# danavery/audio-tokens

Measured on AMD Instinct MI355X. Metric: STFT frames/sec through K-means+tokenize, n_mels=64 vocab=8192, higher is better.
Workload: dtype f32; 1 GPU; configs[3] per-GPU shard x1: 22500+2500 clips/GPU of 10 s @22.05 kHz (43075000 frames/GPU), n_mels=64, vocab_size=8192, niter=20, k-means batches of 10000 files on a 2097152-row subsample; parallelism=dp1

## Files before the change

audio_tokens_amd/_lib.py:

```python
from __future__ import annotations

import ctypes
from pathlib import Path

_PKG = Path(__file__).resolve().parent
LIB_PATH = _PKG / "libaudio_tokens_amd.so"

AT_LAYOUT_MEL_MAJOR = 0
AT_LAYOUT_FRAME_MAJOR = 1

_c = ctypes
_vp, _i32, _i64 = _c.c_void_p, _c.c_int, _c.c_int64

class PrunedArgs(_c.Structure):
    _fields_ = [("x", _vp), ("n", _i64), ("d", _i32), ("c", _vp), ("k", _i32), ("order", _vp), ("hint_sorted", _vp),
                ("cperm", _vp), ("ng", _i32), ("bounds", _vp), ("guess_only", _i32), ("use_filter", _i32),
                ("prepass_done", _i32), ("image_current", _i32), ("ids", _vp), ("dist_or_null", _vp)]


SIGNATURES = {
    "at_version": (_i32, []),
    "at_last_error": (_c.c_char_p, []),
    "at_create": (_i32, [_i32, _c.POINTER(_vp)]),
    "at_destroy": (None, [_vp]),
    "at_workspace_bytes": (_i64, [_vp]),
    "at_background_stream": (_i32, [_vp, _c.POINTER(_vp)]),
    "at_debug_set": (_i32, [_vp, _c.c_char_p, _i32]),
    "at_debug_get": (_i32, [_vp, _c.c_char_p, _c.POINTER(_i32)]),
    "at_diag_errors": (_i32, [_c.POINTER(_i64), _c.POINTER(_i32), _c.POINTER(_i64), _c.POINTER(_i32), _c.c_char_p, _i32, _i32]),
    "at_debug_leave_error_pending": (_i32, []),
    "at_rand_perm_mt19937": (_i32, [_i64, _i64, _vp]),
    "at_rand_perm_prefix_mt19937": (_i32, [_i64, _i64, _i64, _vp]),
    "at_rand_perm_prefix_device": (_i32, [_vp, _i64, _i64, _i64, _vp, _vp]),
    "at_mel_filterbank_host": (_i32, [_i32, _i32, _i32, _vp]),
    "at_num_frames": (_i64, [_i64, _i32]),
    "at_split_clusters_host": (_i32, [_i32, _i32, _i64, _vp, _vp, _c.POINTER(_i32)]),
    "at_logmel_f32": (_i32, [_vp, _vp, _i64, _i64, _i64, _i32, _i32, _i32, _i32, _vp, _vp, _i32, _i32, _vp]),
    "at_resample_length": (_i64, [_i64, _i32, _i32]),
    "at_resample_taps_host": (_i32, [_i32, _i32, _c.POINTER(_i32), _c.POINTER(_i32), _c.POINTER(_i32), _vp, _i64]),
    "at_resample_f32": (_i32, [_vp, _vp, _i64, _i64, _i64, _i32, _i32, _vp, _i64, _vp]),
    "at_minmax_scale_clips_f32": (_i32, [_vp, _vp, _i64, _i64, _vp]),
    "at_conv1d_mel_f32": (_i32, [_vp, _vp, _i64, _i32, _vp, _vp, _i32, _i32, _i32, _vp, _vp]),
    "at_logmel_minmax_f32": (_i32, [_vp, _vp, _i64, _i64, _i64, _i32, _i32, _i32, _i32, _vp, _vp, _i32, _vp]),
    "at_l2norm_rows_f32": (_i32, [_vp, _vp, _i64, _i32, _vp, _vp]),
    "at_assign_f32": (_i32, [_vp, _vp, _i64, _i32, _vp, _i32, _vp, _vp, _vp]),
    "at_assign_hinted_f32": (_i32, [_vp, _vp, _i64, _i32, _vp, _i32, _vp, _vp, _vp, _vp, _vp, _vp]),
    "at_group_rows_kd_host": (_i32, [_vp, _i32, _i32, _i32, _vp]),
    "at_group_min_dist_f32": (_i32, [_vp, _vp, _i32, _i32, _vp, _i32, _vp, _vp]),
    "at_visit_order_f32": (_i32, [_vp, _vp, _vp, _i64, _i32, _vp, _vp, _vp]),
    "at_prune_stats": (_i32, [_vp, _c.POINTER(_i64), _c.POINTER(_i64), _i32]),
    "at_assign_coarse_f32": (_i32, [_vp, _vp, _i64, _i32, _vp, _i32, _vp, _i32, _vp, _vp, _vp, _vp, _vp]),
    "at_filter_stats": (_i32, [_vp, _c.POINTER(_i64), _c.POINTER(_i64), _c.POINTER(_c.c_double), _c.POINTER(_i64),
                               _c.POINTER(_i64), _c.POINTER(_i64), _i32]),
    "at_filter_probe_f32": (_i32, [_vp, _vp, _i64, _i32, _vp, _i32, _vp, _vp, _vp, _i32, _vp, _vp, _vp,
                                   _c.POINTER(_i64), _vp]),
    "at_group_means_f32": (_i32, [_vp, _vp, _i32, _i32, _vp, _i32, _vp, _vp]),
    "at_group_neighbours_f32": (_i32, [_vp, _vp, _i32, _i32, _i32, _vp, _vp]),
    "at_assign_pruned_f32": (_i32, [_vp, _vp, _vp]),
    "at_prune_mask_f32": (_i32, [_vp, _vp, _i64, _i32, _vp, _i32, _vp, _vp, _i32, _vp, _i32, _vp]),
    "at_gather_rows_f32": (_i32, [_vp, _vp, _i32, _vp, _i64, _vp, _vp]),
# ... 90 lines not shown
```

audio_tokens_amd/backend.py:

```python
from __future__ import annotations

import ctypes
import os

import numpy as np
import torch

from . import _lib

_vp = ctypes.c_void_p


def _ptr(t) -> _vp:
    return _vp(t.data_ptr()) if t is not None else _vp(None)


def _np_ptr(a: np.ndarray) -> _vp:
    return _vp(a.ctypes.data)


class HostHelpers:

    def __init__(self):
        self.lib = _lib.load()
# ... 160 lines not shown
        return torch.empty(shape, dtype=dtype).pin_memory()

    def synchronize(self) -> None:
        torch.cuda.current_stream(self.device).synchronize()

    def background_stream(self):
        if getattr(self, "_bg_stream", None) is None:
            h = ctypes.c_void_p()
            _lib.check(self.lib.at_background_stream(self.ctx.handle, ctypes.byref(h)))
            self._bg_stream = torch.cuda.ExternalStream(h.value, device=self.device)
        return self._bg_stream

    def record_event_timed(self):
        ev = torch.cuda.Event(enable_timing=True)
        ev.record(torch.cuda.current_stream(self.device))
        return ev

    def record_event(self):
        ev = torch.cuda.Event()
        ev.record(torch.cuda.current_stream(self.device))
        return ev

    def logmel(self, wave, sample_rate=22050, n_fft=512, hop=128, n_mels=64, fb=None,
               frame_major=False, l2norm=False, out=None) -> torch.Tensor:
        wave = self._f32(wave)
        if wave.dim() == 1:
            wave = wave.unsqueeze(0)
        assert wave.dim() == 2
        n_clips, L = wave.shape
        T = self.num_frames(L, hop)
        fbt = self._f32(fb) if fb is not None else None
        if fbt is not None:
            assert tuple(fbt.shape) == (n_fft // 2 + 1, n_mels), "fb must be [n_fft/2+1, n_mels]"
        shape = (n_clips * T, n_mels) if frame_major else (n_clips, n_mels, T)
        if out is None:
            out = self.empty(shape)
        else:
            assert out.is_contiguous() and out.dtype == torch.float32 and out.numel() == n_clips * T * n_mels
        rec = self._trace_list("logmel")
        if rec is not None:
            e0, e1 = torch.cuda.Event(enable_timing=True), torch.cuda.Event(enable_timing=True)
            e0.record(torch.cuda.current_stream(self.device))
        with torch.cuda.device(self.device):
            _lib.check(self.lib.at_logmel_f32(
                self.ctx.handle, _ptr(wave), n_clips, L, wave.stride(0), sample_rate, n_fft, hop, n_mels,
                _ptr(fbt), _ptr(out), _lib.AT_LAYOUT_FRAME_MAJOR if frame_major else _lib.AT_LAYOUT_MEL_MAJOR,
                1 if l2norm else 0, self._stream()))
        if rec is not None:
            e1.record(torch.cuda.current_stream(self.device))
            rec.append(("logmel", n_clips * T, n_mels, hop, e0, e1))
        return out

    def logmel_minmax(self, wave, sample_rate=22050, n_fft=512, hop=128, n_mels=64, fb=None) -> torch.Tensor:
        wave = self._f32(wave)
        if wave.dim() == 1:
            wave = wave.unsqueeze(0)
        n_clips, L = wave.shape
        T = self.num_frames(L, hop)
        fbt = self._f32(fb) if fb is not None else None
        out = self.empty((n_clips, n_mels, T))
        with torch.cuda.device(self.device):
            for c0 in range(0, n_clips, 65535):
                c1 = min(n_clips, c0 + 65535)
                _lib.check(self.lib.at_logmel_minmax_f32(
                    self.ctx.handle, _ptr(wave[c0:c1]), c1 - c0, L, wave.stride(0), sample_rate, n_fft, hop, n_mels,
                    _ptr(fbt), _ptr(out[c0:c1]), _lib.AT_LAYOUT_MEL_MAJOR, self._stream()))
        return out

    def resample(self, wave, orig_freq: int, new_freq: int) -> torch.Tensor:
        wave = self._f32(wave)
        squeeze = wave.dim() == 1
        if squeeze:
            wave = wave.unsqueeze(0)
# ... 446 lines not shown
```

audio_tokens_amd/csrc/host_group.cpp:

```cpp
#include <algorithm>
#include <cmath>
#include <vector>

#include "at_internal.h"

extern "C" {

int at_group_rows_kd_host(const float* rows, int k, int d, int leaf, int32_t* perm_out) {
    AT_REQUIRE(rows && perm_out && k > 0 && d > 0 && leaf > 0, "at_group_rows_kd_host: bad arguments");
    const int ngroups = (k + leaf - 1) / leaf;
    std::vector<int32_t> idx((size_t)k);
    for (int i = 0; i < k; i++) idx[i] = i;
    struct Part { int lo, hi, g0, g1; };
    std::vector<Part> stack{{0, k, 0, ngroups}};
    std::vector<int> bounds((size_t)ngroups + 1, 0);
    bounds[ngroups] = k;
    std::vector<float> meanf((size_t)d), axisf((size_t)d), nextf((size_t)d), proj((size_t)k), cen;
    while (!stack.empty()) {
        const Part p = stack.back();
        stack.pop_back();
        if (p.g1 - p.g0 <= 1) {
            bounds[p.g0] = p.lo;
            continue;
        }
// ... 9 lines not shown
            const float* r = rows + (size_t)idx[p.lo + i] * d;
            float* c = cen.data() + (size_t)i * d;
            for (int f = 0; f < d; f++) c[f] = r[f] - meanf[f];
        }
        for (int f = 0; f < d; f++) axisf[f] = 1.0f + 0.01f * (float)f;
        for (int it = 0; it < 4; it++) {
            std::fill(nextf.begin(), nextf.end(), 0.0f);
            for (int i = 0; i < m; i++) {
                const float* c = cen.data() + (size_t)i * d;
                float t = 0.0f;
                for (int f = 0; f < d; f++) t += c[f] * axisf[f];
                for (int f = 0; f < d; f++) nextf[f] += t * c[f];
            }
            float nrm = 0.0f;
            for (int f = 0; f < d; f++) nrm += nextf[f] * nextf[f];
            if (!(nrm > 0.0f)) break;
            nrm = 1.0f / std::sqrt(nrm);
            for (int f = 0; f < d; f++) axisf[f] = nextf[f] * nrm;
        }
        for (int i = 0; i < m; i++) {
            const float* c = cen.data() + (size_t)i * d;
            float t = 0.0f;
            for (int f = 0; f < d; f++) t += c[f] * axisf[f];
            proj[idx[p.lo + i]] = t;
        }
        const int gmid = p.g0 + (p.g1 - p.g0) / 2;
        int cut = p.lo + (gmid - p.g0) * leaf;
        if (cut > p.hi) cut = p.hi;
        std::nth_element(idx.begin() + p.lo, idx.begin() + cut, idx.begin() + p.hi, [&](int32_t a, int32_t b) {
            return proj[a] < proj[b] || (proj[a] == proj[b] && a < b);
        });
        stack.push_back({p.lo, cut, p.g0, gmid});
        stack.push_back({cut, p.hi, gmid, p.g1});
    }
    for (int g = 0; g < ngroups; g++) {
        const int lo = bounds[g], hi = bounds[g + 1];
        for (int e = 0; e < leaf; e++) perm_out[(size_t)g * leaf + e] = lo + e < hi ? idx[lo + e] : -1;
    }
    return AT_OK;
}


}
```

audio_tokens_amd/csrc/logmel.hip:

```cpp
#include <cmath>
#include <cstdlib>
#include <cstring>
#include <vector>

#include "at_internal.h"
#include "l2norm_core.h"
#include "logmel_core.h"

namespace {

using namespace logmel;

constexpr int WG = 256;
constexpr int PREFETCH_REGS = 5;
constexpr int TAB_WIN = 0, TAB_TW256 = 512, TAB_TW512 = 1024, TAB_FLOATS = 1536;
constexpr int FRAME_STRIDE = FRAME_LDS_FLOATS + 32;

struct LogmelParams {
    const float* wave;
    long n_clips, L, wave_stride;
    int hop, T, n_mels, fpb;
    long n_blocks;
    int blocks_per_clip;
    const float* tabs;
// ... 204 lines not shown
                    f4 v = {src[0], src[1], src[2], src[3]};
                    if (p.fuse_l2norm) {
                        const float dn = den[f];
#pragma unroll
                        for (int e = 0; e < 4; e++) v[e] = l2n::divide(v[e], dn);
                    }
                    reinterpret_cast<f4*>(dst)[e4] = v;
                }
            } else {
                const int total = nf * p.n_mels;
                for (int e = tid; e < total; e += WG) {
                    const int f = e / p.n_mels, m = e - f * p.n_mels;
                    float v = ostage[f * opitch + m];
                    if (p.fuse_l2norm) v = l2n::divide(v, den[f]);
                    dst[e] = v;
                }
            }
        } else {
            float* dst = p.out + (long)clip * p.n_mels * p.T + t0;
            const int total = p.n_mels * p.fpb;
            for (int e = tid; e < total; e += WG) {
                const int m = e / p.fpb, f = e - m * p.fpb;
                if (f < nf) dst[(long)m * p.T + f] = ostage[f * opitch + m];
            }
        }
    }
}

size_t lds_bytes(int fpb, int hop, int n_mels, size_t fb_ints) {
    const int nsamp = (fpb - 1) * hop + NFFT;
    return sizeof(float) * ((size_t)2 * NFFT + ((nsamp + 3) & ~3) + 16 * FRAME_STRIDE + (size_t)fpb * (n_mels + 1) + fpb) +
           fb_ints * 4 + 16;
}
constexpr size_t LDS_TWO_PER_CU = 80 * 1024;

int build_tables(at_ctx* ctx, int sample_rate, int n_mels, int hop, const float* fb_user_dev, hipStream_t stream,
                 const float** tabs, const int** st, const int** ln, const int** of, const float** wt,
                 int* n_weights, int* quads) {
    bool cached = ctx->ws[WS_LOGMEL_FB] && ctx->fb_sr == sample_rate && ctx->fb_nfft == NFFT &&
                  ctx->fb_nmels == n_mels && (ctx->fb_user != nullptr) == (fb_user_dev != nullptr) && ctx->fb_hop == hop;
    std::vector<float> fb((size_t)NBIN * n_mels);
    if (fb_user_dev) {
        AT_HIP(hipStreamSynchronize(stream));
        AT_HIP(hipMemcpy(fb.data(), fb_user_dev, fb.size() * sizeof(float), hipMemcpyDeviceToHost));
        cached = cached && ctx->fb_user_copy && std::memcmp(ctx->fb_user_copy, fb.data(), fb.size() * sizeof(float)) == 0;
    }
// ... 155 lines not shown
    if (n_clips == 0) return AT_OK;
    AT_REQUIRE(hop >= 1, "at_logmel_minmax_f32: hop=%d out of range", hop);
    const int64_t clip_elems = at_num_frames(L, hop) * n_mels;
    if (n_fft != NFFT) {
        int rc = logmel_impl(ctx, wave, n_clips, L, wave_stride, sample_rate, n_fft, hop, n_mels, fb_or_null, out, layout, 0,
                             nullptr, stream);
        if (rc) return rc;
        return at_minmax_scale_clips_f32(ctx, out, n_clips, clip_elems, stream_);
    }
    AT_REQUIRE(n_clips <= 65535, "at_logmel_minmax_f32: at most 65535 clips per call");
    AT_HIP(hipSetDevice(ctx->device));
    unsigned* mm = static_cast<unsigned*>(at_ws(ctx, WS_LOGMEL_MINMAX, (size_t)n_clips * 16, stream));
    if (!mm) return AT_E_NOMEM;
    AT_LAUNCH(minmax_init_kernel, dim3((unsigned)((n_clips + 255) / 256)), dim3(256), 0, stream, mm, (long)n_clips);
    int rc = logmel_impl(ctx, wave, n_clips, L, wave_stride, sample_rate, n_fft, hop, n_mels, fb_or_null, out, layout, 0, mm,
                         stream);
    if (rc) return rc;
    int bx = (int)((clip_elems + 256 * 8 - 1) / (256 * 8));
    if (bx < 1) bx = 1;
    if (bx > 64) bx = 64;
    AT_LAUNCH(minmax_apply_kernel, dim3((unsigned)bx, (unsigned)n_clips), dim3(256), 0, stream, out, (long)clip_elems, mm);
    return AT_OK;
}
```

audio_tokens_amd/ops.py:

```python
from __future__ import annotations

import collections
import os
import sys
import time
from collections import OrderedDict

import numpy as np
import torch

from .backend import default_backend

__all__ = ["LogMelSpectrogram", "Resample", "Kmeans", "IndexFlatL2", "normalize_rows"]


def _is_host(x) -> bool:
    return isinstance(x, np.ndarray) or (isinstance(x, torch.Tensor) and x.device.type == "cpu")


def normalize_rows(x, backend=None):
    be = backend or default_backend()
    host = _is_host(x)
    y = be.l2norm_rows(x)
    return be.to_host(y) if host else y
# ... 129 lines not shown
class Kmeans:

    def __init__(self, d, k, niter=20, verbose=False, gpu=True, seed=1234, max_points_per_centroid=256,
                 min_points_per_centroid=39, distributed=False, process_group=None, backend=None, **kwargs):
        unsupported = {kk: v for kk, v in kwargs.items() if kk not in ("nredo",) or v != 1}
        if unsupported:
            raise NotImplementedError(f"Kmeans: unsupported ClusteringParameters {sorted(unsupported)}")
        self.d, self.k, self.niter, self.verbose = int(d), int(k), int(niter), bool(verbose)
        self.gpu = gpu
        self.seed = int(seed)
        self.max_points_per_centroid = int(max_points_per_centroid)
        self.min_points_per_centroid = int(min_points_per_centroid)
        self.backend = backend or default_backend()
        self._dist_enabled, self._group = distributed, process_group
        self.centroids_device = None
        self._centroids_host = None
        self._iteration_stats, self._stats_pending = [], None
        self.index = None
        self.phase_seconds = None
        self.prune = True
        self.order_beside = True
        self.exchange = "auto"

    def train(self, x, init_centroids=None, sync=True, check_finite=True):
        be = self.backend
        k, d = self.k, self.d
        dist = _Dist(self._dist_enabled, self._group)
        if isinstance(x, np.ndarray):
            assert x.flags.c_contiguous, "x must be C-contiguous"
        x = be._f32(x)
        assert x.dim() == 2 and x.shape[1] == d, f"expected [n, {d}], got {tuple(x.shape)}"
        n_loc = x.shape[0]
        sizes = dist.all_gather_sizes(n_loc, be.device)
        off = sum(sizes[:dist.rank])
        n = sum(sizes)
        if n < k:
            raise RuntimeError(f"Error: 'nx >= k' failed: Number of training points ({n}) should be at "
                               f"least as large as number of clusters ({k})")
        if check_finite and dist.any_flag(be.any_nonfinite(x) if n_loc else False, be.device):
            raise RuntimeError("Error: 'std::isfinite(x_in[i])' failed: input contains NaN's or Inf's")

        if n > k * self.max_points_per_centroid:
            ns = k * self.max_points_per_centroid
            if self.verbose:
                print(f"Sampling a subset of {ns} / {n} for training")
            perm = self._subsample_perm(n, ns)
            if dist.on:
                mine = (perm >= off) & (perm < off + n_loc)
                pos = torch.nonzero(mine).reshape(-1)
                xs = be.gather_rows(x, (perm[mine] - off).to(torch.int32).contiguous())
            else:
                pos = None
                xs = be.gather_rows(x, perm)
        else:
            ns = n
            if ns < k * self.min_points_per_centroid:
                print(f"WARNING clustering {ns} points to {k} centroids: please provide at least "
                      f"{k * self.min_points_per_centroid} training points", file=sys.stderr)
            xs = x
            pos = off + torch.arange(n_loc, dtype=torch.int64, device=x.device) if dist.on else None

        def rows_at(positions):
            positions = np.asarray(positions, dtype=np.int64)
            if not dist.on:
                return be.gather_rows(xs, positions.astype(np.int32))
            out = be.zeros((len(positions), d))
            want = be.from_host(positions)
            if pos.numel():
                j = torch.searchsorted(pos, want).clamp_(max=pos.numel() - 1)
                ok = pos[j] == want
                if bool(ok.any()):
                    out[ok] = be.gather_rows(xs, j[ok].to(torch.int32).contiguous())
            return dist.sum_bits(out)

        self._stats_pending = None
        self._iteration_stats = []
        if ns == k:
# ... 126 lines not shown
                be.split_clusters_device(hassign, cent, ns, nsplit_dev[it:it + 1])
            tp = lap("exchange+finalize+split", tp)
            if prune and timed_events:
                paced.append(be.record_event_timed())
                if len(paced) > 3:
                    done = paced.popleft()
                    done.synchronize()
                    if last_done is not None:
                        iter_ms = last_done.elapsed_time(done)
                    last_done = done
        self._last_assign = ids
        self._stats_pending = (stats_dev[:niter], nsplit_dev[:niter], t0)
        if self.verbose:
            for it, st in enumerate(self.iteration_stats):
                print(f"  Iteration {it} ({st['time']:.2f} s, search {st['time_search']:.2f} s): "
                      f"objective={st['obj']:g} imbalance={st['imbalance_factor']:.3f} nsplit={st['nsplit']}", flush=True)
        if prune:
            if regrouping is not None and (regrouping.done() or regrouping_is_late):
                cperm = upload(regrouping.result())
            self._cperm_cache = ((k, d), cperm)
            self._grouping_of_result = cperm
        return self._finish(cent, sync)

    def _subsample_perm(self, n, m):
        key = (int(n), self.seed, int(m))
        cache = self.__dict__.setdefault("_perm_cache", OrderedDict())
        hit = cache.get(key)
        if hit is None:
            hit = cache[key] = self.backend.rand_perm_prefix_device(n, self.seed, m)
            while len(cache) > 2:
                cache.popitem(last=False)
        return hit

    def _read_stats(self, stats_dev, nsplit_dev, t0):
        be = self.backend
        st, ns = be.to_host(stats_dev), be.to_host(nsplit_dev)
        if (ns < 0).any():
            raise RuntimeError("Kmeans: split_clusters found no donor (every cluster has at most one point)")
        el = time.time() - t0
        return [dict(obj=float(np.float32(st[i, 0])), time=el * (i + 1) / len(ns), time_search=el * (i + 1) / len(ns),
                     imbalance_factor=float(st[i, 1]), nsplit=int(ns[i])) for i in range(len(ns))]

    @property
    def iteration_stats(self):
        if self._stats_pending is not None:
            self._iteration_stats = self._read_stats(*self._stats_pending)
# ... 108 lines not shown
```

audio_tokens_amd/pipeline.py:

```python
from __future__ import annotations

import os
import time
from dataclasses import dataclass, field

import torch

from .backend import default_backend
from .ops import IndexFlatL2, Kmeans


@dataclass
class PipelineResult:
    centroids: torch.Tensor
    tokens_train: torch.Tensor
    tokens_val: torch.Tensor
    frames_per_clip: int
    stage_seconds: dict = field(default_factory=dict)
    kmeans_stats: list = field(default_factory=list)


class DevicePipeline:
    def __init__(self, n_mels=64, vocab_size=500, niter=20, sample_rate=22050, n_fft=512, hop_length=128,
                 clustering_batch_size=10000, spectrogram_batch_size=5000, distributed=False,
                 process_group=None, backend=None, verbose=False, prune=True):
        self.n_mels, self.vocab_size, self.niter = n_mels, vocab_size, niter
        self.sample_rate, self.n_fft, self.hop_length = sample_rate, n_fft, hop_length
        self.clustering_batch_size = clustering_batch_size
        self.spectrogram_batch_size = spectrogram_batch_size
        self.distributed, self.process_group = distributed, process_group
        self.be = backend or default_backend()
        self.verbose = verbose
        self.prune = prune
        self.overlap_logmel = os.environ.get("AT_OVERLAP_LOGMEL", "1") != "0"
        self.beside_clips = int(os.environ.get("AT_BESIDE_CLIPS", "50"))
        self.world = 1
        if distributed:
            import torch.distributed as dist
            if dist.is_initialized():
                self.world = dist.get_world_size(process_group)

    def _frames(self, wave):
        be = self.be
        n_clips, L = wave.shape
        T = be.num_frames(L, self.hop_length)
        out = be.empty((n_clips * T, self.n_mels))
        step = self.spectrogram_batch_size
        for c0 in range(0, n_clips, step):
            c1 = min(n_clips, c0 + step)
            be.logmel(wave[c0:c1], self.sample_rate, self.n_fft, self.hop_length, self.n_mels,
                      frame_major=True, l2norm=True, out=out[c0 * T:c1 * T])
        return out, T

    def _frames_beside(self, wave_tr, wave_va, per_rank):
        be = self.be
        n_clips, L = wave_tr.shape
        T = be.num_frames(L, self.hop_length)
        main = torch.cuda.current_stream(be.device)
        if getattr(self, "_lm_stream", None) is None:
            self._lm_stream = be.background_stream() if os.environ.get("AT_BESIDE_PRIO", "1") != "0" else torch.cuda.Stream(device=be.device)
        side = self._lm_stream
        frames_tr = be.empty((n_clips * T, self.n_mels))
        n_va = 0 if wave_va is None else wave_va.shape[0]
        frames_va = be.empty((n_va * T, self.n_mels)) if n_va else None
        take_flag = hasattr(be, "logmel_nonfinite_take")
        if take_flag:
            be.logmel_nonfinite_take()

        def logmel(wave, frames, c0, c1):
            be.logmel(wave[c0:c1], self.sample_rate, self.n_fft, self.hop_length, self.n_mels, frame_major=True, l2norm=True,
                      out=frames[c0 * T:c1 * T])

        first = min(n_clips, per_rank)
        for c0 in range(0, first, self.spectrogram_batch_size):
            logmel(wave_tr, frames_tr, c0, min(first, c0 + self.spectrogram_batch_size))
        ready = [torch.cuda.Event()]
        ready[0].record(main)
        piece = self.beside_clips
        bad = None
        with torch.cuda.stream(side):
            side.wait_event(ready[0])
            for b0 in range(first, n_clips, per_rank):
                b1 = min(n_clips, b0 + per_rank)
                for c0 in range(b0, b1, piece):
                    logmel(wave_tr, frames_tr, c0, min(b1, c0 + piece))
                ev = torch.cuda.Event()
                ev.record(side)
                ready.append(ev)
            if take_flag:
                bad = be.logmel_nonfinite_take()
            for c0 in range(0, n_va, piece):
                logmel(wave_va, frames_va, c0, min(n_va, c0 + piece))
            done = torch.cuda.Event()
            done.record(side)
        return frames_tr, frames_va, T, ready, done, bad

    def overlaps_logmel(self, n_train_clips) -> bool:
        per_rank = max(1, self.clustering_batch_size // self.world)
        return (self.overlap_logmel and self.be.device.type == "cuda" and n_train_clips > per_rank and self.prune
                and self.vocab_size >= 1024 and self.n_mels in (64, 128))

    def run(self, wave_train, wave_val=None, timing=False) -> PipelineResult:
        be = self.be
        sync = be.synchronize if timing else (lambda: None)
        secs = {}
        per_rank = max(1, self.clustering_batch_size // self.world)

        t0 = time.perf_counter()
        take_flag = hasattr(be, "logmel_nonfinite_take")
        beside = not timing and self.overlaps_logmel(wave_train.shape[0])
        ready = done = None
        if beside:
            frames_tr, frames_va, T, ready, done, bad = self._frames_beside(
                be._f32(wave_train), be._f32(wave_val) if wave_val is not None and wave_val.shape[0] > 0 else None, per_rank)
        else:
            if take_flag:
                be.logmel_nonfinite_take()
            frames_tr, T = self._frames(be._f32(wave_train))
            bad = be.logmel_nonfinite_take() if take_flag else None
            frames_va = None
            if wave_val is not None and wave_val.shape[0] > 0:
                frames_va, _ = self._frames(be._f32(wave_val))
        sync(); secs["logmel"] = time.perf_counter() - t0

        t0 = time.perf_counter()
        km = Kmeans(self.n_mels, self.vocab_size, niter=self.niter, verbose=self.verbose,
                    distributed=self.distributed, process_group=self.process_group, backend=be)
        km.prune = self.prune
        n_clips = wave_train.shape[0]
        pending = []
        if bad is None:
            if done is not None:
                torch.cuda.current_stream(be.device).wait_event(done)
            bad = be.nonfinite_flag(frames_tr)
        for b, c0 in enumerate(range(0, n_clips, per_rank)):
            c1 = min(n_clips, c0 + per_rank)
            x = frames_tr[c0 * T:c1 * T]
            if ready is not None:
                torch.cuda.current_stream(be.device).wait_event(ready[b])
            km.train(x, init_centroids=None if b == 0 else km.centroids_device, sync=False, check_finite=False)
            pending.append(km._stats_pending)
        centroids = be.l2norm_rows(km.centroids_device)
        km.lend_grouping(centroids)
        sync(); secs["kmeans"] = time.perf_counter() - t0

        t0 = time.perf_counter()
        index = IndexFlatL2(self.n_mels, backend=be)
        index.prune = self.prune
        index.add(centroids)
        if done is not None:
            torch.cuda.current_stream(be.device).wait_event(done)
        tok_tr, _ = index.assign(frames_tr, want_dist=False)
        tok_va = be.empty((0,), torch.int64)
        if frames_va is not None:
            tok_va, _ = index.assign(frames_va, want_dist=False)
        sync(); secs["tokenize"] = time.perf_counter() - t0

        def over_ranks(flag):
            if self.world > 1:
                import torch.distributed as dist
                flag = flag.cpu() if dist.get_backend(self.process_group) == "gloo" else flag
                dist.all_reduce(flag, op=dist.ReduceOp.MAX, group=self.process_group)
            return bool(flag.item())

        if over_ranks(bad):
            if not take_flag or over_ranks(be.nonfinite_flag(frames_tr)):
                raise RuntimeError("Error: 'std::isfinite(x_in[i])' failed: input contains NaN's or Inf's")
        stats = [km._read_stats(*p) for p in pending if p is not None]
        return PipelineResult(centroids, tok_tr, tok_va, T, secs, stats)

    class _Feeder:

        def __init__(self, be, wave_host, chunk_clips):
            self.be, self.wave, self.chunk = be, wave_host, int(chunk_clips)
            L = wave_host.shape[1]
            self.pinned = wave_host.is_pinned()
            self.copy_stream = torch.cuda.Stream(device=be.device)
            self.dev = [torch.empty((self.chunk, L), dtype=torch.float32, device=be.device) for _ in range(2)]
            self.stage = None if self.pinned else [torch.empty((self.chunk, L), dtype=torch.float32).pin_memory()
# ... 84 lines not shown
```

include/audio_tokens_amd.h:

```cpp
#ifndef AUDIO_TOKENS_AMD_H
#define AUDIO_TOKENS_AMD_H

#include <stdint.h>

#ifdef __cplusplus
extern "C" {
#endif

#define AT_VERSION 100

#define AT_OK 0
#define AT_E_INVALID (-1)
#define AT_E_HIP (-2)
#define AT_E_NOMEM (-3)
#define AT_E_TOO_FEW (-4)
#define AT_E_NONFINITE (-5)
#define AT_E_COMM (-6)

#define AT_LAYOUT_MEL_MAJOR 0
#define AT_LAYOUT_FRAME_MAJOR 1

typedef struct at_ctx at_ctx;

int at_version(void);
const char* at_last_error(void);
int at_create(int device, at_ctx** out);
void at_destroy(at_ctx* ctx);
int64_t at_workspace_bytes(const at_ctx* ctx);
int at_background_stream(at_ctx* ctx, void** stream_out);

int at_rand_perm_mt19937(int64_t n, int64_t seed, int32_t* perm_host);
int at_rand_perm_prefix_mt19937(int64_t n, int64_t seed, int64_t m, int32_t* prefix_host);
int at_mel_filterbank_host(int sample_rate, int n_fft, int n_mels, float* fb_host);
int64_t at_num_frames(int64_t L, int hop);
int at_split_clusters_host(int d, int k, int64_t n, float* hassign_host, float* centroids_host,
                           int* nsplit);

int at_logmel_f32(at_ctx* ctx, const float* wave, int64_t n_clips, int64_t L, int64_t wave_stride,
                  int sample_rate, int n_fft, int hop, int n_mels, const float* fb_or_null,
                  float* out, int layout, int fuse_l2norm, void* stream);

int64_t at_resample_length(int64_t L, int orig_freq, int new_freq);
int at_resample_taps_host(int orig_freq, int new_freq, int* orig_out, int* new_out, int* width_out,
                          float* taps_host, int64_t taps_capacity);
int at_resample_f32(at_ctx* ctx, const float* wave, int64_t n_clips, int64_t L, int64_t wave_stride,
                    int orig_freq, int new_freq, float* out, int64_t out_stride, void* stream);

int at_l2norm_rows_f32(at_ctx* ctx, const float* x, int64_t n, int d, float* y, void* stream);

int at_minmax_scale_clips_f32(at_ctx* ctx, float* x, int64_t n_clips, int64_t clip_elems, void* stream);

int at_conv1d_mel_f32(at_ctx* ctx, const float* x, int64_t n, int n_mels, const float* weight, const float* bias_or_null,
                      int num_kernels, int kernel_size, int padding, float* out, void* stream);

int at_logmel_minmax_f32(at_ctx* ctx, const float* wave, int64_t n_clips, int64_t L, int64_t wave_stride,
                         int sample_rate, int n_fft, int hop, int n_mels, const float* fb_or_null,
                         float* out, int layout, void* stream);

int at_assign_f32(at_ctx* ctx, const float* x, int64_t n, int d, const float* c, int k,
                  int64_t* ids, float* dist_or_null, void* stream);

int at_assign_hinted_f32(at_ctx* ctx, const float* x, int64_t n, int d, const float* c, int k,
                         const int64_t* hint_ids_or_null, const uint32_t* order_or_null,
// ... 88 lines not shown
```

Before: 278.8 million frames/s.

## Compute log-mel only for subsampled k-means rows first, overlap the rest

Adds a logmel_rows kernel that computes log-mel frames only for the randomly subsampled row indices, so the first k-means batch can start training before the full-batch log-mel finishes. The remaining log-mel work is scheduled on a side stream in pieces and flushed lazily, with events fencing k-means batches and tokenization. The intent is to take log-mel off the critical path. In exchange it recomputes the STFT for the subsampled rows and adds scheduling complexity. It also clamps non-finite projections in host grouping.

```diff
diff --git a/audio_tokens_amd/_lib.py b/audio_tokens_amd/_lib.py
--- a/audio_tokens_amd/_lib.py
+++ b/audio_tokens_amd/_lib.py
@@ -36,6 +36,8 @@
     "at_num_frames": (_i64, [_i64, _i32]),
     "at_split_clusters_host": (_i32, [_i32, _i32, _i64, _vp, _vp, _c.POINTER(_i32)]),
     "at_logmel_f32": (_i32, [_vp, _vp, _i64, _i64, _i64, _i32, _i32, _i32, _i32, _vp, _vp, _i32, _i32, _vp]),
+    "at_logmel_pieces_f32": (_i32, [_vp, _vp, _i64, _i64, _i64, _i32, _i32, _i32, _i32, _vp, _vp, _i32, _i64, _vp]),
+    "at_logmel_rows_f32": (_i32, [_vp, _vp, _i64, _i64, _i64, _i32, _i32, _i32, _i32, _vp, _vp, _i64, _vp, _vp]),
     "at_resample_length": (_i64, [_i64, _i32, _i32]),
     "at_resample_taps_host": (_i32, [_i32, _i32, _c.POINTER(_i32), _c.POINTER(_i32), _c.POINTER(_i32), _vp, _i64]),
     "at_resample_f32": (_i32, [_vp, _vp, _i64, _i64, _i64, _i32, _i32, _vp, _i64, _vp]),
diff --git a/audio_tokens_amd/backend.py b/audio_tokens_amd/backend.py
--- a/audio_tokens_amd/backend.py
+++ b/audio_tokens_amd/backend.py
@@ -206,7 +206,7 @@
         return ev
 
     def logmel(self, wave, sample_rate=22050, n_fft=512, hop=128, n_mels=64, fb=None,
-               frame_major=False, l2norm=False, out=None) -> torch.Tensor:
+               frame_major=False, l2norm=False, out=None, piece_clips=None) -> torch.Tensor:
         wave = self._f32(wave)
         if wave.dim() == 1:
             wave = wave.unsqueeze(0)
@@ -226,13 +226,40 @@
             e0, e1 = torch.cuda.Event(enable_timing=True), torch.cuda.Event(enable_timing=True)
             e0.record(torch.cuda.current_stream(self.device))
         with torch.cuda.device(self.device):
-            _lib.check(self.lib.at_logmel_f32(
-                self.ctx.handle, _ptr(wave), n_clips, L, wave.stride(0), sample_rate, n_fft, hop, n_mels,
-                _ptr(fbt), _ptr(out), _lib.AT_LAYOUT_FRAME_MAJOR if frame_major else _lib.AT_LAYOUT_MEL_MAJOR,
-                1 if l2norm else 0, self._stream()))
+            if piece_clips is not None:
+                assert frame_major, "piece_clips: frame-major layout only"
+                _lib.check(self.lib.at_logmel_pieces_f32(
+                    self.ctx.handle, _ptr(wave), n_clips, L, wave.stride(0), sample_rate, n_fft, hop, n_mels, _ptr(fbt),
+                    _ptr(out), 1 if l2norm else 0, int(piece_clips), self._stream()))
+            else:
+                _lib.check(self.lib.at_logmel_f32(
+                    self.ctx.handle, _ptr(wave), n_clips, L, wave.stride(0), sample_rate, n_fft, hop, n_mels,
+                    _ptr(fbt), _ptr(out), _lib.AT_LAYOUT_FRAME_MAJOR if frame_major else _lib.AT_LAYOUT_MEL_MAJOR,
+                    1 if l2norm else 0, self._stream()))
         if rec is not None:
             e1.record(torch.cuda.current_stream(self.device))
             rec.append(("logmel", n_clips * T, n_mels, hop, e0, e1))
+        return out
+
+    def logmel_rows(self, wave, rows, sample_rate=22050, n_fft=512, hop=128, n_mels=64, fb=None, out=None) -> torch.Tensor:
+        wave = self._f32(wave)
+        if wave.dim() == 1:
+            wave = wave.unsqueeze(0)
+        assert wave.dim() == 2 and wave.stride(1) == 1
+        assert rows.dtype == torch.int32 and rows.is_contiguous() and rows.device == self.device
+        n_clips, L = wave.shape
+        m = rows.numel()
+        fbt = self._f32(fb) if fb is not None else None
+        if fbt is not None:
+            assert tuple(fbt.shape) == (n_fft // 2 + 1, n_mels), "fb must be [n_fft/2+1, n_mels]"
+        if out is None:
+            out = self.empty((m, n_mels))
+        else:
+            assert out.is_contiguous() and out.dtype == torch.float32 and tuple(out.shape) == (m, n_mels)
+        with torch.cuda.device(self.device):
+            _lib.check(self.lib.at_logmel_rows_f32(
+                self.ctx.handle, _ptr(wave), n_clips, L, wave.stride(0), sample_rate, n_fft, hop, n_mels, _ptr(fbt),
+                _ptr(rows), m, _ptr(out), self._stream()))
         return out
 
     def logmel_minmax(self, wave, sample_rate=22050, n_fft=512, hop=128, n_mels=64, fb=None) -> torch.Tensor:
diff --git a/audio_tokens_amd/csrc/host_group.cpp b/audio_tokens_amd/csrc/host_group.cpp
--- a/audio_tokens_amd/csrc/host_group.cpp
+++ b/audio_tokens_amd/csrc/host_group.cpp
@@ -1,4 +1,5 @@
 #include <algorithm>
+#include <cfloat>
 #include <cmath>
 #include <vector>
 
@@ -55,7 +56,7 @@
             const float* c = cen.data() + (size_t)i * d;
             float t = 0.0f;
             for (int f = 0; f < d; f++) t += c[f] * axisf[f];
-            proj[idx[p.lo + i]] = t;
+            proj[idx[p.lo + i]] = std::isfinite(t) ? t : FLT_MAX;
         }
         const int gmid = p.g0 + (p.g1 - p.g0) / 2;
         int cut = p.lo + (gmid - p.g0) * leaf;
diff --git a/audio_tokens_amd/csrc/logmel.hip b/audio_tokens_amd/csrc/logmel.hip
--- a/audio_tokens_amd/csrc/logmel.hip
+++ b/audio_tokens_amd/csrc/logmel.hip
@@ -250,6 +250,142 @@
             for (int e = tid; e < total; e += WG) {
                 const int m = e / p.fpb, f = e - m * p.fpb;
                 if (f < nf) dst[(long)m * p.T + f] = ostage[f * opitch + m];
+            }
+        }
+    }
+}
+
+struct LogmelRowsParams {
+    const float* wave;
+    long L, wave_stride, n_frames;
+    int hop, T, n_mels;
+    const int* rows;
+    long m, n_groups;
+    const float* tabs;
+    const int* fb_start;
+    const int* fb_len;
+    const int* fb_off;
+    const float* fb_wts;
+    int fb_nw, fb_lds, fb_quads;
+    float* out;
+};
+
+constexpr int ROWS_PER_GROUP = 16;
+
+size_t rows_lds_bytes(int n_mels, size_t fb_ints) {
+    return sizeof(float) * ((size_t)2 * NFFT + 16 * FRAME_STRIDE + (size_t)ROWS_PER_GROUP * (n_mels + 1) + ROWS_PER_GROUP) +
+           fb_ints * 4 + 16;
+}
+
+__global__ void __launch_bounds__(WG, 2) logmel_rows_kernel(LogmelRowsParams p) {
+    extern __shared__ __attribute__((aligned(16))) float sm[];
+    const int tid = threadIdx.x, lane = tid & 63, wave = tid >> 6;
+    const int l16 = lane & 15, grp = lane >> 4;
+    const int opitch = p.n_mels + 1;
+
+    float* win = sm;
+    float* tw512 = win + NFFT;
+    float* work = tw512 + NFFT;
+    float* ostage = work + 16 * FRAME_STRIDE;
+    float* den = ostage + ROWS_PER_GROUP * opitch;
+    int* fbi = reinterpret_cast<int*>(sm + ((2 * NFFT + 16 * FRAME_STRIDE + ROWS_PER_GROUP * opitch + ROWS_PER_GROUP + 3) & ~3));
+    const int* fb_start = p.fb_start;
+    const int* fb_len = p.fb_len;
+    const int* fb_off = p.fb_off;
+    const float* fb_wts = p.fb_wts;
+    if (p.fb_lds) {
+        const int nint = (3 * p.n_mels + 3) & ~3;
+        for (int i = tid; i < nint + p.fb_nw; i += WG) fbi[i] = p.fb_start[i];
+        fb_start = fbi;
+        fb_len = fbi + p.n_mels;
+        fb_off = fbi + 2 * p.n_mels;
+        fb_wts = reinterpret_cast<const float*>(fbi + nint);
+    }
+    cpx twr[16];
+#pragma unroll
+    for (int k1 = 0; k1 < 16; k1++)
+        twr[k1] = {p.tabs[TAB_TW256 + 2 * (k1 * 16 + l16)], p.tabs[TAB_TW256 + 2 * (k1 * 16 + l16) + 1]};
+    for (int i = tid; i < NFFT; i += WG) {
+        win[i] = p.tabs[TAB_WIN + i];
+        tw512[i] = p.tabs[TAB_TW512 + i];
+    }
+
+    const int f = wave * 4 + grp;
+    float* mybuf = work + f * FRAME_STRIDE;
+    const int n_mel_iter = (p.n_mels + 15) >> 4;
+
+    for (long g = blockIdx.x; g < p.n_groups; g += gridDim.x) {
+        __syncthreads();
+        const long i = g * ROWS_PER_GROUP + f;
+        const long r = i < p.m ? (long)p.rows[i] : 0;
+        const bool valid = r >= 0 && r < p.n_frames;
+        const long rr = valid ? r : 0;
+        const long clip = rr / p.T;
+        const int t = (int)(rr - clip * p.T);
+        const float* w = p.wave + clip * p.wave_stride;
+        const long s0 = (long)t * p.hop - NFFT / 2;
+        const float* frame = w + s0;
+        if (!(s0 >= 0 && s0 + NFFT <= p.L)) {
+            for (int j = 0; j < NFFT / 16; j++) {
+                long q = s0 + l16 + 16 * j;
+                if (q < 0) q = -q;
+                if (q >= p.L) q = 2 * (p.L - 1) - q;
+                if (q < 0) q = 0;
+                if (q >= p.L) q = p.L - 1;
+                mybuf[l16 + 16 * j] = w[q];
+            }
+            frame = mybuf;
+        }
+        __builtin_amdgcn_wave_barrier();
+
+        phase1_w(l16, frame, win, twr, mybuf);
+        cpx z[16];
+        phase2(l16, mybuf, z);
+        phase3_publish(l16, z, mybuf);
+        float pw[16], p256 = 0.0f;
+        phase3_power(l16, z, mybuf, tw512, pw, p256);
+#pragma unroll
+        for (int e = 0; e < 16; e++) mybuf[l16 + 16 * e] = pw[e];
+        if (l16 < 4) mybuf[256 + l16] = l16 == 0 ? p256 : 0.0f;
+        for (int k = 0; k < n_mel_iter; k++) {
+            const int m = l16 + 16 * k;
+            if (m < p.n_mels) {
+                const float s = p.fb_quads ? mel_band(mybuf, fb_start[m], fb_len[m], fb_wts + fb_off[m])
+                                           : mel_band_plain(mybuf, fb_start[m], fb_len[m], fb_wts + fb_off[m]);
+                ostage[f * opitch + m] = !(s <= 1e-10f) ? 3.0102999566398120f * __builtin_amdgcn_logf(s) : -100.0f;
+            }
+        }
+        if (l16 == 0) den[f] = valid ? 0.0f : __builtin_nanf("");
+        __syncthreads();
+
+        const long i0 = g * ROWS_PER_GROUP;
+        const int nf = (int)min((long)ROWS_PER_GROUP, p.m - i0);
+        {
+            const int ff = tid >> 3;
+            if (ff < ROWS_PER_GROUP) {
+                const float ss = l2n::pairwise_sumsq_8lanes(ostage + ff * opitch, p.n_mels, tid & 7);
+                if ((tid & 7) == 0 && den[ff] == 0.0f) den[ff] = __builtin_sqrtf(ss) + 1e-10f;
+            }
+        }
+        __syncthreads();
+        float* dst = p.out + i0 * p.n_mels;
+        if ((p.n_mels & 3) == 0 && (reinterpret_cast<uintptr_t>(dst) & 15) == 0) {
+            typedef float f4 __attribute__((ext_vector_type(4)));
+            const int mq = p.n_mels >> 2, total4 = nf * mq;
+            for (int e4 = tid; e4 < total4; e4 += WG) {
+                const int ff = e4 / mq, m = (e4 - ff * mq) * 4;
+                const float* src = ostage + ff * opitch + m;
+                f4 v = {src[0], src[1], src[2], src[3]};
+                const float dn = den[ff];
+#pragma unroll
+                for (int e = 0; e < 4; e++) v[e] = l2n::divide(v[e], dn);
+                reinterpret_cast<f4*>(dst)[e4] = v;
+            }
+        } else {
+            const int total = nf * p.n_mels;
+            for (int e = tid; e < total; e += WG) {
+                const int ff = e / p.n_mels, m = e - ff * p.n_mels;
+                dst[e] = l2n::divide(ostage[ff * opitch + m], den[ff]);
             }
         }
     }
@@ -451,3 +587,62 @@
     AT_LAUNCH(minmax_apply_kernel, dim3((unsigned)bx, (unsigned)n_clips), dim3(256), 0, stream, out, (long)clip_elems, mm);
     return AT_OK;
 }
+
+extern "C" int at_logmel_rows_f32(at_ctx* ctx, const float* wave, int64_t n_clips, int64_t L, int64_t wave_stride,
+                                  int sample_rate, int n_fft, int hop, int n_mels, const float* fb_or_null,
+                                  const int32_t* rows, int64_t m, float* out, void* stream_) {
+    hipStream_t stream = (hipStream_t)stream_;
+    AT_REQUIRE(ctx, "at_logmel_rows_f32: ctx is null");
+    AT_REQUIRE(n_fft == NFFT, "at_logmel_rows_f32: n_fft=%d not supported (512 only)", n_fft);
+    AT_REQUIRE(hop >= 1 && hop <= n_fft, "at_logmel_rows_f32: hop=%d out of range [1, %d]", hop, n_fft);
+    AT_REQUIRE(n_mels >= 8 && n_mels <= 128, "at_logmel_rows_f32: n_mels=%d out of range [8, 128]", n_mels);
+    AT_REQUIRE(n_clips >= 0 && m >= 0, "at_logmel_rows_f32: negative size");
+    AT_REQUIRE(L > n_fft / 2, "at_logmel_rows_f32: clip length %lld must exceed n_fft/2 (reflect padding)", (long long)L);
+    AT_REQUIRE(wave_stride >= L, "at_logmel_rows_f32: wave_stride < L");
+    if (m == 0) return AT_OK;
+    AT_REQUIRE(n_clips > 0, "at_logmel_rows_f32: rows of no clips");
+    AT_REQUIRE(wave && rows && out, "at_logmel_rows_f32: null pointer");
+    AT_HIP(hipSetDevice(ctx->device));
+    const int64_t T = at_num_frames(L, hop);
+    AT_REQUIRE(T < (1LL << 31), "at_logmel_rows_f32: too many frames per clip");
+
+    LogmelRowsParams p;
+    int rc = build_tables(ctx, sample_rate, n_mels, hop, fb_or_null, stream, &p.tabs, &p.fb_start, &p.fb_len,
+                          &p.fb_off, &p.fb_wts, &p.fb_nw, &p.fb_quads);
+    if (rc) return rc;
+    p.wave = wave; p.L = L; p.wave_stride = wave_stride; p.n_frames = n_clips * T;
+    p.hop = hop; p.T = (int)T; p.n_mels = n_mels;
+    p.rows = rows; p.m = m; p.n_groups = (m + ROWS_PER_GROUP - 1) / ROWS_PER_GROUP;
+    p.out = out;
+    const size_t fb_ints = (((size_t)3 * n_mels + 3) & ~(size_t)3) + p.fb_nw;
+    p.fb_lds = fb_ints * 4 <= 14 * 1024;
+    const size_t lds = rows_lds_bytes(n_mels, p.fb_lds ? fb_ints : 0);
+    AT_REQUIRE(lds <= 160 * 1024, "at_logmel_rows_f32: n_mels=%d needs %zu bytes of LDS", n_mels, lds);
+    { const int rcl_ = at_raise_lds(ctx, reinterpret_cast<const void*>(&logmel_rows_kernel), lds); if (rcl_) return rcl_; }
+    int per_cu = 0;
+    AT_HIP(hipOccupancyMaxActiveBlocksPerMultiprocessor(&per_cu, reinterpret_cast<const void*>(&logmel_rows_kernel), WG, lds));
+    if (per_cu < 1) per_cu = 1;
+    long grid = (long)per_cu * ctx->n_cus;
+    if (grid > p.n_groups) grid = p.n_groups;
+    AT_LAUNCH(logmel_rows_kernel, dim3((unsigned)grid), dim3(WG), lds, stream, p);
+    return AT_OK;
+}
+
+extern "C" int at_logmel_pieces_f32(at_ctx* ctx, const float* wave, int64_t n_clips, int64_t L, int64_t wave_stride,
+                                    int sample_rate, int n_fft, int hop, int n_mels, const float* fb_or_null, float* out,
+                                    int fuse_l2norm, int64_t piece_clips, void* stream_) {
+    AT_REQUIRE(ctx, "at_logmel_pieces_f32: ctx is null");
+    AT_REQUIRE(piece_clips >= 1, "at_logmel_pieces_f32: piece_clips=%lld must be positive", (long long)piece_clips);
+    AT_REQUIRE(n_clips >= 0, "at_logmel_pieces_f32: n_clips out of range");
+    AT_REQUIRE(hop >= 1 && hop <= n_fft, "at_logmel_pieces_f32: hop=%d out of range [1, %d]", hop, n_fft);
+    AT_REQUIRE(L > n_fft / 2, "at_logmel_pieces_f32: clip length %lld must exceed n_fft/2 (reflect padding)", (long long)L);
+    AT_REQUIRE(wave_stride >= L, "at_logmel_pieces_f32: wave_stride < L");
+    const int64_t piece_floats = at_num_frames(L, hop) * n_mels;
+    for (int64_t c0 = 0; c0 < n_clips; c0 += piece_clips) {
+        const int64_t n = n_clips - c0 < piece_clips ? n_clips - c0 : piece_clips;
+        const int rc = logmel_impl(ctx, wave + c0 * wave_stride, n, L, wave_stride, sample_rate, n_fft, hop, n_mels, fb_or_null,
+                                   out + c0 * piece_floats, AT_LAYOUT_FRAME_MAJOR, fuse_l2norm, nullptr, (hipStream_t)stream_);
+        if (rc) return rc;
+    }
+    return AT_OK;
+}
diff --git a/audio_tokens_amd/ops.py b/audio_tokens_amd/ops.py
--- a/audio_tokens_amd/ops.py
+++ b/audio_tokens_amd/ops.py
@@ -175,7 +175,9 @@
         self.order_beside = True
         self.exchange = "auto"
 
-    def train(self, x, init_centroids=None, sync=True, check_finite=True):
+    def train(self, x, init_centroids=None, sync=True, check_finite=True, rows_of=None, wait_x=None):
+        if rows_of is not None:
+            assert wait_x is not None, "rows_of needs wait_x (x is read directly when there is no subsample)"
         be = self.backend
         k, d = self.k, self.d
         dist = _Dist(self._dist_enabled, self._group)
@@ -190,10 +192,12 @@
         if n < k:
             raise RuntimeError(f"Error: 'nx >= k' failed: Number of training points ({n}) should be at "
                                f"least as large as number of clusters ({k})")
+        if check_finite and wait_x is not None:
+            wait_x()
         if check_finite and dist.any_flag(be.any_nonfinite(x) if n_loc else False, be.device):
             raise RuntimeError("Error: 'std::isfinite(x_in[i])' failed: input contains NaN's or Inf's")
 
-        if n > k * self.max_points_per_centroid:
+        if self.subsamples(n):
             ns = k * self.max_points_per_centroid
             if self.verbose:
                 print(f"Sampling a subset of {ns} / {n} for training")
@@ -201,11 +205,14 @@
             if dist.on:
                 mine = (perm >= off) & (perm < off + n_loc)
                 pos = torch.nonzero(mine).reshape(-1)
-                xs = be.gather_rows(x, (perm[mine] - off).to(torch.int32).contiguous())
+                mine_idx = (perm[mine] - off).to(torch.int32).contiguous()
+                xs = be.gather_rows(x, mine_idx) if rows_of is None else rows_of(mine_idx)
             else:
                 pos = None
-                xs = be.gather_rows(x, perm)
+                xs = be.gather_rows(x, perm) if rows_of is None else rows_of(perm)
         else:
+            if wait_x is not None and not check_finite:
+                wait_x()
             ns = n
             if ns < k * self.min_points_per_centroid:
                 print(f"WARNING clustering {ns} points to {k} centroids: please provide at least "
@@ -378,6 +385,9 @@
             self._grouping_of_result = cperm
         return self._finish(cent, sync)
 
+    def subsamples(self, n) -> bool:
+        return n > self.k * self.max_points_per_centroid
+
     def _subsample_perm(self, n, m):
         key = (int(n), self.seed, int(m))
         cache = self.__dict__.setdefault("_perm_cache", OrderedDict())
diff --git a/audio_tokens_amd/pipeline.py b/audio_tokens_amd/pipeline.py
--- a/audio_tokens_amd/pipeline.py
+++ b/audio_tokens_amd/pipeline.py
@@ -34,6 +34,7 @@
         self.prune = prune
         self.overlap_logmel = os.environ.get("AT_OVERLAP_LOGMEL", "1") != "0"
         self.beside_clips = int(os.environ.get("AT_BESIDE_CLIPS", "50"))
+        self.subsample_first = os.environ.get("AT_SUBSAMPLE_FIRST", "1") != "0"
         self.world = 1
         if distributed:
             import torch.distributed as dist
@@ -52,48 +53,76 @@
                       frame_major=True, l2norm=True, out=out[c0 * T:c1 * T])
         return out, T
 
-    def _frames_beside(self, wave_tr, wave_va, per_rank):
-        be = self.be
-        n_clips, L = wave_tr.shape
-        T = be.num_frames(L, self.hop_length)
-        main = torch.cuda.current_stream(be.device)
-        if getattr(self, "_lm_stream", None) is None:
-            self._lm_stream = be.background_stream() if os.environ.get("AT_BESIDE_PRIO", "1") != "0" else torch.cuda.Stream(device=be.device)
-        side = self._lm_stream
-        frames_tr = be.empty((n_clips * T, self.n_mels))
-        n_va = 0 if wave_va is None else wave_va.shape[0]
-        frames_va = be.empty((n_va * T, self.n_mels)) if n_va else None
-        take_flag = hasattr(be, "logmel_nonfinite_take")
-        if take_flag:
-            be.logmel_nonfinite_take()
-
-        def logmel(wave, frames, c0, c1):
-            be.logmel(wave[c0:c1], self.sample_rate, self.n_fft, self.hop_length, self.n_mels, frame_major=True, l2norm=True,
-                      out=frames[c0 * T:c1 * T])
-
-        first = min(n_clips, per_rank)
-        for c0 in range(0, first, self.spectrogram_batch_size):
-            logmel(wave_tr, frames_tr, c0, min(first, c0 + self.spectrogram_batch_size))
-        ready = [torch.cuda.Event()]
-        ready[0].record(main)
-        piece = self.beside_clips
-        bad = None
-        with torch.cuda.stream(side):
-            side.wait_event(ready[0])
-            for b0 in range(first, n_clips, per_rank):
-                b1 = min(n_clips, b0 + per_rank)
-                for c0 in range(b0, b1, piece):
-                    logmel(wave_tr, frames_tr, c0, min(b1, c0 + piece))
-                ev = torch.cuda.Event()
-                ev.record(side)
-                ready.append(ev)
-            if take_flag:
-                bad = be.logmel_nonfinite_take()
-            for c0 in range(0, n_va, piece):
-                logmel(wave_va, frames_va, c0, min(n_va, c0 + piece))
-            done = torch.cuda.Event()
-            done.record(side)
-        return frames_tr, frames_va, T, ready, done, bad
+    class _Beside:
+
+        def __init__(self, pipe, wave_tr, wave_va, per_rank, subsample_first):
+            be = self.be = pipe.be
+            n_clips, L = wave_tr.shape
+            T = self.T = be.num_frames(L, pipe.hop_length)
+            self.main = torch.cuda.current_stream(be.device)
+            if getattr(pipe, "_lm_stream", None) is None:
+                pipe._lm_stream = (be.background_stream() if os.environ.get("AT_BESIDE_PRIO", "1") != "0"
+                                   else torch.cuda.Stream(device=be.device))
+            self.side = pipe._lm_stream
+            self.frames_tr = be.empty((n_clips * T, pipe.n_mels))
+            n_va = 0 if wave_va is None else wave_va.shape[0]
+            self.frames_va = be.empty((n_va * T, pipe.n_mels)) if n_va else None
+            self.take_flag = hasattr(be, "logmel_nonfinite_take")
+            if self.take_flag:
+                be.logmel_nonfinite_take()
+            self.piece = pipe.beside_clips
+            self.args = (pipe.sample_rate, pipe.n_fft, pipe.hop_length, pipe.n_mels)
+            batches = [(b0, min(n_clips, b0 + per_rank)) for b0 in range(0, n_clips, per_rank)]
+            order = list(range(len(batches)))
+            if subsample_first:
+                order = order[1:] + order[:1]
+            else:
+                first = batches[0][1]
+                for c0 in range(0, first, pipe.spectrogram_batch_size):
+                    self._logmel(wave_tr, self.frames_tr, c0, min(first, c0 + pipe.spectrogram_batch_size))
+                order = order[1:]
+            start = torch.cuda.Event()
+            start.record(self.main)
+            self.side.wait_event(start)
+            self.ready = [start] * len(batches)
+            self.todo = [[wave_tr, self.frames_tr, batches[b][0], batches[b][1], b] for b in order]
+            self.todo.append([wave_tr, self.frames_tr, 0, 0, "take"])
+            self.todo.append([wave_va, self.frames_va, 0, n_va, "done"])
+            self.bad = self.done = None
+            self.flushed = set() if subsample_first else {0}
+
+        def _logmel(self, wave, frames, c0, c1, piece=None):
+            T = self.T
+            self.be.logmel(wave[c0:c1], *self.args, frame_major=True, l2norm=True, out=frames[c0 * T:c1 * T],
+                           piece_clips=piece)
+
+        def _mark(self, marker):
+            if marker == "take":
+                self.bad = self.be.logmel_nonfinite_take() if self.take_flag else None
+                return
+            ev = torch.cuda.Event()
+            ev.record(self.side)
+            if marker == "done":
+                self.done = ev
+            else:
+                self.ready[marker] = ev
+            self.flushed.add(marker)
+
+        def flush_to(self, marker):
+            with torch.cuda.stream(self.side):
+                while self.todo and marker not in self.flushed:
+                    wave, frames, c0, c1, mark = self.todo.pop(0)
+                    if c0 < c1:
+                        self._logmel(wave, frames, c0, c1, self.piece)
+                    self._mark(mark)
+
+        def fence(self):
+            ev = torch.cuda.Event()
+            ev.record(self.side)
+            self.main.wait_event(ev)
+
+    def _rows_kernel_covers(self) -> bool:
+        return hasattr(self.be, "logmel_rows") and self.n_fft == 512 and 8 <= self.n_mels <= 128
 
     def overlaps_logmel(self, n_train_clips) -> bool:
         per_rank = max(1, self.clustering_batch_size // self.world)
@@ -109,52 +138,79 @@
         t0 = time.perf_counter()
         take_flag = hasattr(be, "logmel_nonfinite_take")
         beside = not timing and self.overlaps_logmel(wave_train.shape[0])
-        ready = done = None
-        if beside:
-            frames_tr, frames_va, T, ready, done, bad = self._frames_beside(
-                be._f32(wave_train), be._f32(wave_val) if wave_val is not None and wave_val.shape[0] > 0 else None, per_rank)
-        else:
-            if take_flag:
-                be.logmel_nonfinite_take()
-            frames_tr, T = self._frames(be._f32(wave_train))
-            bad = be.logmel_nonfinite_take() if take_flag else None
-            frames_va = None
-            if wave_val is not None and wave_val.shape[0] > 0:
-                frames_va, _ = self._frames(be._f32(wave_val))
-        sync(); secs["logmel"] = time.perf_counter() - t0
-
-        t0 = time.perf_counter()
         km = Kmeans(self.n_mels, self.vocab_size, niter=self.niter, verbose=self.verbose,
                     distributed=self.distributed, process_group=self.process_group, backend=be)
         km.prune = self.prune
         n_clips = wave_train.shape[0]
-        pending = []
-        if bad is None:
-            if done is not None:
-                torch.cuda.current_stream(be.device).wait_event(done)
-            bad = be.nonfinite_flag(frames_tr)
-        for b, c0 in enumerate(range(0, n_clips, per_rank)):
-            c1 = min(n_clips, c0 + per_rank)
-            x = frames_tr[c0 * T:c1 * T]
-            if ready is not None:
-                torch.cuda.current_stream(be.device).wait_event(ready[b])
-            km.train(x, init_centroids=None if b == 0 else km.centroids_device, sync=False, check_finite=False)
-            pending.append(km._stats_pending)
-        centroids = be.l2norm_rows(km.centroids_device)
-        km.lend_grouping(centroids)
-        sync(); secs["kmeans"] = time.perf_counter() - t0
-
-        t0 = time.perf_counter()
-        index = IndexFlatL2(self.n_mels, backend=be)
-        index.prune = self.prune
-        index.add(centroids)
-        if done is not None:
-            torch.cuda.current_stream(be.device).wait_event(done)
-        tok_tr, _ = index.assign(frames_tr, want_dist=False)
-        tok_va = be.empty((0,), torch.int64)
-        if frames_va is not None:
-            tok_va, _ = index.assign(frames_va, want_dist=False)
-        sync(); secs["tokenize"] = time.perf_counter() - t0
+        T0 = be.num_frames(wave_train.shape[1], self.hop_length)
+        sub_first = (beside and self.subsample_first and self._rows_kernel_covers()
+                     and km.subsamples(min(n_clips, per_rank) * T0 * self.world))
+        wave_tr = be._f32(wave_train)
+        wave_va = be._f32(wave_val) if wave_val is not None and wave_val.shape[0] > 0 else None
+        bs = None
+        if beside:
+            bs = self._Beside(self, wave_tr, wave_va, per_rank, sub_first)
+            frames_tr, frames_va, T, bad = bs.frames_tr, bs.frames_va, bs.T, None
+        else:
+            if take_flag:
+                be.logmel_nonfinite_take()
+            frames_tr, T = self._frames(wave_tr)
+            bad = be.logmel_nonfinite_take() if take_flag else None
+            frames_va = None
+            if wave_va is not None:
+                frames_va, _ = self._frames(wave_va)
+        sync(); secs["logmel"] = time.perf_counter() - t0
+
+        main = torch.cuda.current_stream(be.device)
+        try:
+            t0 = time.perf_counter()
+            pending = []
+            if bs is not None and not bs.take_flag:
+                bs.flush_to("done")
+                main.wait_event(bs.done)
+                bad = be.nonfinite_flag(frames_tr)
+            elif bad is None and not take_flag:
+                bad = be.nonfinite_flag(frames_tr)
+            if bs is not None:
+                bs.flush_to("done")
+            for b, c0 in enumerate(range(0, n_clips, per_rank)):
+                c1 = min(n_clips, c0 + per_rank)
+                x = frames_tr[c0 * T:c1 * T]
+                rows_of = wait_x = None
+                if bs is not None:
+                    def wait_x(b=b):
+                        bs.flush_to(b)
+                        main.wait_event(bs.ready[b])
+                    if sub_first and b == 0:
+                        rows_of = (lambda idx, w=wave_tr[c0:c1]: be.logmel_rows(
+                            w, idx, self.sample_rate, self.n_fft, self.hop_length, self.n_mels))
+                    else:
+                        wait_x()
+                        wait_x = None
+                km.train(x, init_centroids=None if b == 0 else km.centroids_device, sync=False, check_finite=False,
+                         rows_of=rows_of, wait_x=wait_x)
+                pending.append(km._stats_pending)
+            centroids = be.l2norm_rows(km.centroids_device)
+            km.lend_grouping(centroids)
+            sync(); secs["kmeans"] = time.perf_counter() - t0
+
+            t0 = time.perf_counter()
+            index = IndexFlatL2(self.n_mels, backend=be)
+            index.prune = self.prune
+            index.add(centroids)
+            if bs is not None:
+                bs.flush_to("done")
+                main.wait_event(bs.done)
+                if bad is None:
+                    bad = bs.bad
+            tok_tr, _ = index.assign(frames_tr, want_dist=False)
+            tok_va = be.empty((0,), torch.int64)
+            if frames_va is not None:
+                tok_va, _ = index.assign(frames_va, want_dist=False)
+            sync(); secs["tokenize"] = time.perf_counter() - t0
+        finally:
+            if bs is not None:
+                bs.fence()
 
         def over_ranks(flag):
             if self.world > 1:
diff --git a/include/audio_tokens_amd.h b/include/audio_tokens_amd.h
--- a/include/audio_tokens_amd.h
+++ b/include/audio_tokens_amd.h
@@ -39,6 +39,14 @@
 int at_logmel_f32(at_ctx* ctx, const float* wave, int64_t n_clips, int64_t L, int64_t wave_stride,
                   int sample_rate, int n_fft, int hop, int n_mels, const float* fb_or_null,
                   float* out, int layout, int fuse_l2norm, void* stream);
+
+int at_logmel_pieces_f32(at_ctx* ctx, const float* wave, int64_t n_clips, int64_t L, int64_t wave_stride,
+                         int sample_rate, int n_fft, int hop, int n_mels, const float* fb_or_null,
+                         float* out, int fuse_l2norm, int64_t piece_clips, void* stream);
+
+int at_logmel_rows_f32(at_ctx* ctx, const float* wave, int64_t n_clips, int64_t L, int64_t wave_stride,
+                       int sample_rate, int n_fft, int hop, int n_mels, const float* fb_or_null,
+                       const int32_t* rows, int64_t m, float* out, void* stream);
 
 int64_t at_resample_length(int64_t L, int orig_freq, int new_freq);
 int at_resample_taps_host(int orig_freq, int new_freq, int* orig_out, int* new_out, int* width_out,
```

Result: faster. 283.7 million frames/s (median of 6 runs) (+1.8%).
